# zerenluo123/legged_gym

Hardware: AMD Instinct MI355X
Metric: env-steps/sec (whole node), Go1 rough-terrain 4096 envs/GPU at 1/2/4/8 GPUs (higher is better)
Workload: dtype fp32; 1 GPU; C3 go1_rough: Go1 trimesh curriculum terrain + 187-point height scan, actuator-net history+MLP, PPO 24 steps x 4096 envs/GPU, 5 epochs x 4 minibatches; envs_per_gpu=4096, global_envs=4096, parallelism=dp1

## Files before the change

legged_gym_amd/csrc/lgx_api.hip:

```cpp
#include <math.h>
#include <stddef.h>
#include <stdio.h>
#include <string.h>

#include <new>
#include <string>
#include <vector>

#include "lgx_internal.h"

static thread_local std::string g_err;

static int fail(int code, const char* msg) {
  g_err = msg;
  return code;
}
static int hip_check(hipError_t e, const char* what) {
  if (e == hipSuccess) return 0;
  char buf[256];
  snprintf(buf, sizeof buf, "%s: %s", what, hipGetErrorString(e));
  g_err = buf;
  return LGX_EHIP;
}
int lgx_fail(int code, const char* msg) { return fail(code, msg); }
int lgx_hip_status(const char* what) { return hip_check(hipGetLastError(), what); }
static int launch_check(int rc, const char* what) {
  if (rc == 0) return 0;
  if (rc == -1) return fail(LGX_EINVAL, what);
  return hip_check(hipGetLastError(), what);
}

struct lgx_sim {
  int device;
  bool dense;
  int pp;
  int act_mode;
  int32_t num_points;
  lgx_env_params params;
  lgx_buffers bufs;
  lgx_dev_model* d_model;
  lgx_env_params* d_params;
  const float* draws;
  float* extras_snapshot;
  lgx_priv_args priv;
  lgx_hist_args hist;
  lgx_act_rand_args arand;
  lgx_cmdcur_args ccur;
  hipStream_t aux;
  hipEvent_t aux_in, aux_done;
  bool aux_pending;
  int32_t n_term_rows;
  int32_t profiling;
  int64_t prof_calls;
  std::vector<hipEvent_t> ev[3];
  std::vector<hipEvent_t> pool;
};

static hipEvent_t take_event(lgx_sim* s) {
  if (!s->pool.empty()) { hipEvent_t e = s->pool.back(); s->pool.pop_back(); return e; }
  hipEvent_t e = nullptr;
  if (hipEventCreateWithFlags(&e, hipEventDisableSystemFence) != hipSuccess) return nullptr;
  return e;
}
thread_local lgx_timing_slot lgx_timing;

static int scratch_zeroed(void** slot, size_t bytes, const char* who, const char* what) {
  const std::string w(who), of = std::string("(") + what + ")";
  const bool fresh = !*slot;
  int rc = fresh ? hip_check(hipMalloc(slot, bytes), (w + ": hipMalloc" + of).c_str()) : 0;
// ... 104 lines not shown
  for (int i = 0; i < (dense ? 0 : model->num_points); ++i) {
    int d = model->point_dyn[i];
    int rep = model->point_report[i];
    if (d < 0 || d >= LGX_NUM_DYN) return fail(LGX_EINVAL, "lgx_sim_create: bad point_dyn");
    int lane;
    if (d == 0) {
      if (rep != 0) return fail(LGX_EINVAL, "lgx_sim_create: base points must report on body 0");
      lane = rr++ & 3;
    } else {
      lane = (d - 1) / 3;
      if (rep < 1 + 4 * lane || rep > 4 + 4 * lane) return fail(LGX_EINVAL, "lgx_sim_create: leg point reports on a foreign body");
    }
    if (dm.lane_npts[lane] >= LGX_MAX_LANE_PTS) return fail(LGX_EINVAL, "lgx_sim_create: too many contact points per leg");
    dm.lane_pts[lane][dm.lane_npts[lane]++] = i;
  }
  for (int l = 0; l < 4; ++l) dm.max_lane_npts = dm.lane_npts[l] > dm.max_lane_npts ? dm.lane_npts[l] : dm.max_lane_npts;
  dm.joint_rot_eye = 1;
  for (int j = 0; j < LGX_NUM_DOF; ++j)
    for (int i = 0; i < 9; ++i)
      if (model->joint_rot[j][i] != (i % 4 == 0 ? 1.f : 0.f)) dm.joint_rot_eye = 0;

  int rc = hip_check(hipSetDevice(device), "hipSetDevice");
  if (rc) return rc;
  lgx_sim* s = new (std::nothrow) lgx_sim();
  if (!s) return fail(LGX_ENOMEM, "lgx_sim_create: out of host memory");
  s->device = device;
  s->dense = dense;
  s->pp = lgx_physics_pp(params->num_envs);
  const char* am = getenv("LGX_ACT_OVERLAP");
  s->act_mode = am && *am ? atoi(am) : 2;
  if (s->act_mode < 0 || s->act_mode > 2 || (am && *am && (am[0] < '0' || am[0] > '2' || am[1]))) {
    delete s;
    return fail(LGX_EINVAL, "lgx_sim_create: LGX_ACT_OVERLAP must be 0, 1 or 2");
  }
  s->num_points = model->num_points;
  s->params = *params;
  s->bufs = *bufs;
  s->draws = nullptr;
  s->extras_snapshot = nullptr;
  s->priv = lgx_priv_args{};
  s->hist = lgx_hist_args{};
  s->arand = lgx_act_rand_args{};
  s->ccur = lgx_cmdcur_args{};
  s->aux = nullptr;
  s->aux_in = s->aux_done = nullptr;
  s->aux_pending = false;
  s->profiling = 0;
  s->prof_calls = 0;
  s->n_term_rows = params->num_terms + (params->termination_slot >= 0 ? 1 : 0);
  if ((rc = hip_check(hipMalloc(&s->d_model, sizeof(lgx_dev_model)), "hipMalloc(model)"))) { delete s; return rc; }
  if ((rc = hip_check(hipMalloc(&s->d_params, sizeof(lgx_env_params)), "hipMalloc(params)"))) {
    (void)hipFree(s->d_model); delete s; return rc;
  }
  rc = hip_check(hipMemcpy(s->d_model, &dm, sizeof dm, hipMemcpyHostToDevice), "hipMemcpy(model)");
  if (!rc) rc = hip_check(hipMemcpy(s->d_params, params, sizeof *params, hipMemcpyHostToDevice), "hipMemcpy(params)");
  if (!rc) {
    const int64_t blocks = (params->num_envs + LGX_ENV_BLOCK - 1) / LGX_ENV_BLOCK;
    rc = hip_check(hipMemset(bufs->scratch + blocks * LGX_PARTIAL_STRIDE, 0, sizeof(unsigned int)), "hipMemset(ticket)");
  }
  if (rc) { (void)hipFree(s->d_model); (void)hipFree(s->d_params); delete s; return rc; }
  *out = s;
  return 0;
}

int lgx_sim_destroy(lgx_sim* s) {
  if (!s) return 0;
// ... 238 lines not shown
    pa.n = s->params.num_envs;
    pa.tag = 0u;
    pa.obs = s->bufs.obs;
    pa.hist = s->hist.row;
    pa.hist_width = s->hist.width;
    pa.priv = s->priv.buf;
    pa.priv_width = s->priv.width;
  }
  const int32_t nblocks = (pa.n + LGX_ENV_BLOCK - 1) / LGX_ENV_BLOCK;
  return launch_check(lgx_launch_cmd_curriculum(s->d_params, s->bufs.scratch, nblocks, s->n_term_rows, s->ccur, pa, st),
                      "command curriculum: launch");
}

int lgx_rebind_extras(lgx_sim* s, float* snapshot) {
  if (!s) return fail(LGX_EINVAL, "lgx_rebind_extras: null sim");
  s->extras_snapshot = snapshot;
  return 0;
}

static int join_aux(lgx_sim* s, hipStream_t st) {
  if (!s->aux_pending) return 0;
  return hip_check(hipStreamWaitEvent(st, s->aux_done, 0), "hipStreamWaitEvent(aux)");
}


int lgx_sync_aux(lgx_sim* s, void* stream) {
  if (!s) return fail(LGX_EINVAL, "lgx_sync_aux: null sim");
  return join_aux(s, (hipStream_t)stream);
}

static int physics(lgx_sim* s, int32_t nsub, int32_t from_actions, const float* actions, hipStream_t st, int32_t frozen) {
  if (s->arand.prev)
    return lgx_launch_physics_rand(s->d_model, s->d_params, s->bufs, s->params.num_envs, nsub, from_actions, actions,
                                   st, frozen, s->pp, s->arand);
  return s->dense ? lgx_launch_physics_dense(s->d_model, s->d_params, s->bufs, s->params.num_envs, nsub, from_actions,
                                             actions, st, frozen, s->num_points)
                  : lgx_launch_physics(s->d_model, s->d_params, s->bufs, s->params.num_envs, nsub, from_actions, actions,
                                       st, frozen, s->pp);
}

int lgx_simulate(lgx_sim* s, int32_t n, void* stream) {
  if (!s || n < 0) return fail(LGX_EINVAL, "lgx_simulate: bad arguments");
  if (n == 0) return 0;
  if (int rc = join_aux(s, (hipStream_t)stream)) return rc;
  return launch_check(physics(s, n, 0, nullptr, (hipStream_t)stream, 0), "lgx_simulate: physics launch");
}

int lgx_drive_inputs(lgx_sim* s, const float* actions, void* stream) {
  if (!s) return fail(LGX_EINVAL, "lgx_drive_inputs: null sim");
  if (int rc = join_aux(s, (hipStream_t)stream)) return rc;
  return launch_check(physics(s, s->params.decimation, 1, actions, (hipStream_t)stream, 1), "lgx_drive_inputs: launch");
}

int lgx_ground_contact(lgx_sim* s, const float* points, int32_t n, float* out, void* stream) {
  if (!s || n < 0 || (n > 0 && (!points || !out))) return fail(LGX_EINVAL, "lgx_ground_contact: bad arguments");
  return launch_check(lgx_launch_ground_contact(s->d_params, s->bufs, points, n, out, (hipStream_t)stream),
                      "lgx_ground_contact: launch");
}

int lgx_post_physics(lgx_sim* s, int64_t step, void* stream) {
  if (!s) return fail(LGX_EINVAL, "lgx_post_physics: null sim");
  if (int rc = launch_check(lgx_launch_post_physics(s->d_params, s->bufs, s->params.num_envs, step, s->draws,
                                                    s->extras_snapshot, nullptr, s->priv, s->hist, (hipStream_t)stream),
                            "lgx_post_physics: launch"))
    return rc;
  return command_curriculum(s, step, (hipStream_t)stream, nullptr, 0);
}

static int post_physics_fused(lgx_sim* s, int64_t step, hipStream_t st, bool sample);

int lgx_step(lgx_sim* s, int64_t step, void* stream) { return lgx_step_from(s, nullptr, step, stream); }
// ... 203 lines not shown
```

legged_gym_amd/csrc/lgx_internal.h:

```cpp
#pragma once
#include <hip/hip_ext.h>
#include <hip/hip_runtime.h>

#include "../../include/lgx.h"

#define LGX_MAX_LANE_PTS 24

struct lgx_dev_model {
  lgx_model m;
  int32_t lane_npts[4];
  int32_t max_lane_npts;
  int32_t joint_rot_eye;
  int32_t lane_pts[4][LGX_MAX_LANE_PTS];
  int32_t pad_tail[(4 - (sizeof(lgx_model) / 4 + 6 + 4 * LGX_MAX_LANE_PTS) % 4) % 4];
};

int lgx_launch_ground_contact(const lgx_env_params* dp, const lgx_buffers& b, const float* q, int32_t n, float* o,
                              hipStream_t stream);
int lgx_physics_pp(int32_t n_envs);
int lgx_launch_physics(const lgx_dev_model* dm, const lgx_env_params* dp, const lgx_buffers& b, int32_t n_envs,
                       int32_t nsub, int32_t from_actions, const float* act_src, hipStream_t stream, int32_t frozen,
                       int pp);
struct lgx_act_rand_args {
  const float* kp_scale;
  const float* kd_scale;
  const int32_t* lag;
  float* prev;
};
int lgx_launch_physics_rand(const lgx_dev_model* dm, const lgx_env_params* dp, const lgx_buffers& b, int32_t n_envs,
                            int32_t nsub, int32_t from_actions, const float* act_src, hipStream_t stream,
                            int32_t frozen, int pp, const lgx_act_rand_args& ar);
int lgx_launch_physics_dense(const lgx_dev_model* dm, const lgx_env_params* dp, const lgx_buffers& b, int32_t n_envs,
                             int32_t nsub, int32_t from_actions, const float* act_src, hipStream_t stream,
                             int32_t frozen, int32_t num_points);
struct lgx_priv_args {
  float* buf;
  int32_t width, num_terms;
  uint32_t ids;
  uint32_t pad;
  uint64_t offs_lo, offs_hi;
  float cf_scale, tq_scale;
  __host__ __device__ int id(int t) const { return (int)((ids >> (4 * t)) & 15u); }
  __host__ __device__ int off(int t) const { return (int)(((t < 4 ? offs_lo : offs_hi) >> (16 * (t & 3))) & 0xffffu); }
  void set(int t, int id_, int off_) {
    ids |= (uint32_t)id_ << (4 * t);
    (t < 4 ? offs_lo : offs_hi) |= (uint64_t)off_ << (16 * (t & 3));
  }
};
static_assert(LGX_PRIV_MAX_TERMS <= 8 && LGX_PRIV_COUNT <= 16 && LGX_MAX_PRIV_OBS < 65536, "lgx_priv_args packing");
struct lgx_hist_args {
  float* row;
  const float* prev;
  int32_t* age;
  int32_t frames, frame_width, width;
};
struct lgx_act_launch {
  const float* in;
  float* out;
  int64_t rows;
  const float* w;
  const float* scale;
};
int lgx_launch_post_physics(const lgx_env_params* dp, const lgx_buffers& b, int32_t n_envs, int64_t step,
                            const float* draws, float* extras_snapshot, const lgx_act_launch* act,
// ... 90 lines not shown
```

legged_gym_amd/csrc/lgx_physics.hip:

```cpp
#include <stdlib.h>

#include "lgx_device.h"
#include "lgx_internal.h"

namespace {

struct sv { f3 a, l; };
LGX_DEV sv sv0() { return sv{mk3(0, 0, 0), mk3(0, 0, 0)}; }
LGX_DEV sv add(sv x, sv y) { return sv{x.a + y.a, x.l + y.l}; }
LGX_DEV sv scale(float s, sv x) { return sv{s * x.a, s * x.l}; }
LGX_DEV float dot(sv x, sv y) { return dot(x.a, y.a) + dot(x.l, y.l); }
LGX_DEV sv crm(sv V, sv s) { return sv{cross(V.a, s.a), cross(V.a, s.l) + cross(V.l, s.a)}; }
LGX_DEV sv crf(sv V, sv f) { return sv{cross(V.a, f.a) + cross(V.l, f.l), cross(V.a, f.l)}; }

struct SI { float m; f3 h; float I[6]; };
LGX_DEV SI si_add(const SI& x, const SI& y) {
  SI r; r.m = x.m + y.m; r.h = x.h + y.h;
#pragma unroll
  for (int i = 0; i < 6; ++i) r.I[i] = x.I[i] + y.I[i];
  return r;
}
LGX_DEV sv si_mul(const SI& s, sv v) {
  f3 Ia = mk3(s.I[0] * v.a.x + s.I[3] * v.a.y + s.I[4] * v.a.z, s.I[3] * v.a.x + s.I[1] * v.a.y + s.I[5] * v.a.z,
              s.I[4] * v.a.x + s.I[5] * v.a.y + s.I[2] * v.a.z);
// ... 355 lines not shown
    const int w0 = w[0], w1 = w[LGX_HF_PATCH], w2 = w[1], w3 = w[LGX_HF_PATCH + 1];
    h[0] = w0 >> 8; h[1] = w1 >> 8; h[2] = w2 >> 8; h[3] = w3 >> 8;
    code[0] = w0 & 15; code[1] = w1 & 15; code[2] = w2 & 15; code[3] = w3 & 15;
  } else {
#pragma unroll
    for (int k = 0; k < 4; ++k) {
      const int64_t o = (int64_t)(ci + (k & 1)) * cols + cj + (k >> 1);
      h[k] = B.height_samples[o];
      code[k] = B.hf_trimesh[o];
    }
#pragma unroll
    for (int k = 0; k < 4; ++k) code[k] &= 15;
  }
  f3 v[4];
#pragma unroll
  for (int k = 0; k < 4; ++k) {
    const int da = ca + (k & 1), db = cb + (k >> 1);
    const int dx = ((code[k] * 11) >> 5) - 1, dy = code[k] - 3 * (dx + 1) - 1;
    v[k] = mk3((float)(da - 1 + dx) * hs, (float)(db - 1 + dy) * hs, (float)h[k] * vs);
  }
  const float zmax = fmaxf(fmaxf(v[0].z, v[1].z), fmaxf(v[2].z, v[3].z));
  const float xmin = fminf(fminf(v[0].x, v[1].x), fminf(v[2].x, v[3].x)), xmax = fmaxf(fmaxf(v[0].x, v[1].x), fmaxf(v[2].x, v[3].x));
  const float ymin = fminf(fminf(v[0].y, v[1].y), fminf(v[2].y, v[3].y)), ymax = fmaxf(fmaxf(v[0].y, v[1].y), fmaxf(v[2].y, v[3].y));
  if (p.z - r > zmax || p.x < xmin - r || p.x > xmax + r || p.y < ymin - r || p.y > ymax + r) return;
  tm_tri(q, p, v[0], v[3], v[2]);
  tm_tri(q, p, v[0], v[1], v[3]);
}

LGX_DEV void tm_init(TmQuery& q, f3 p) {
  q.d2 = 3.0e38f; q.cp = p; q.cn = mk3(0.f, 0.f, 1.f);
  q.top = -3.0e38f; q.tn = mk3(0.f, 0.f, 1.f);
}

LGX_DEV float tm_finish(const TmQuery& q, f3 p, float r, f3* n) {
  const bool inside = p.z < q.top;
  const float d = sqrtf(q.d2);
  if (d > 1e-7f) {
    const float inv = ph_rcp(d);
    *n = inside ? inv * (q.cp - p) : inv * (p - q.cp);
  } else {
    f3 c = q.top > -1e30f ? q.tn : q.cn;
    c = (c.z < 0.f ? -1.f : 1.f) / fmaxf(sqrtf(dot(c, c)), 1e-30f) * c;
    *n = c;
  }
  return inside ? r + d : r - d;
}

LGX_DEV bool tm_near(const lgx_env_params* __restrict__ P, const lgx_buffers& B, f3 p, float r, int i, int j,
                     const int32_t* hpatch, int pi0, int pj0) {
  int hv[16], cd[16];
  tm_block(B, i, j, hpatch, pi0, pj0, hv, cd);
  int hmax = hv[0];
#pragma unroll
  for (int k = 1; k < 16; ++k) hmax = max(hmax, hv[k]);
  return !(p.z - r > (float)hmax * P->vertical_scale);
}

LGX_DEV unsigned tm_keep(const lgx_env_params* __restrict__ P, const lgx_buffers& B, f3 p, float r, int i, int j,
                         const int32_t* hpatch, int pi0, int pj0, f3* pl) {
  const float hs = P->horizontal_scale, vs = P->vertical_scale;
  const int rows = B.hf_rows, cols = B.hf_cols;
  int hv[16], cd[16];
  tm_block(B, i, j, hpatch, pi0, pj0, hv, cd);
  int hmax = hv[0];
#pragma unroll
  for (int k = 1; k < 16; ++k) hmax = max(hmax, hv[k]);
// ... 84 lines not shown
              h11 = (float)(q11 >> 8) * vs;
  const float fu = clampf(u - (float)i, 0.f, 1.f), fv = clampf(v - (float)j, 0.f, 1.f);
  float gx, gy, h;
  if (fu >= fv) { gx = (h10 - h00) * ihs; gy = (h11 - h10) * ihs; h = h00 + fu * (h10 - h00) + fv * (h11 - h10); }
  else          { gx = (h11 - h01) * ihs; gy = (h01 - h00) * ihs; h = h00 + fv * (h01 - h00) + fu * (h11 - h01); }
  const float inv = ph_rsqrt(gx * gx + gy * gy + 1.0f);
  *n = mk3(-gx * inv, -gy * inv, inv);
  return (h - p.z) * n->z + r;
}

LGX_DEV float ground_contact(const lgx_env_params* __restrict__ P, const lgx_buffers& B, f3 p, float r, f3* n,
                             const int32_t* patch, int pi0, int pj0) {
  bool defer;
  const float d = ground_cell(P, B, p, r, n, patch, pi0, pj0, &defer);
  if (!defer) return d;
  int i, j;
  tm_cell(P, B, p, &i, &j);
  return trimesh_depth(P, B, p, r, i, j, n, patch, pi0, pj0);
}

LGX_DEV void wave_lds_sync() {
  __builtin_amdgcn_fence(__ATOMIC_RELEASE, "wavefront");
  __builtin_amdgcn_wave_barrier();
  __builtin_amdgcn_fence(__ATOMIC_ACQUIRE, "wavefront");
}

}

#define MAX_LANE_PTS LGX_MAX_LANE_PTS
#ifndef LGX_PHYS_WAVES_PER_SIMD
#define LGX_PHYS_WAVES_PER_SIMD 1
#endif
#define HIST_STRIDE 31

template <int PP>
LGX_DEV float psum(float v) {
  if (PP == 4) return row_quads_sum(v);
  if (PP >= 2) v += lane_xor4(v);
  if (PP >= 4) v += lane_xor8(v);
  if (PP >= 8) v += __shfl_xor(v, 16);
  return v;
}

#define PHYS_KP(k, j) (RAND ? arow[k] : M->kp[j])
#define PHYS_KD(k, j) (RAND ? arow[3 + (k)] : M->kd[j])
#define PHYS_PG(k, j) (RAND ? arow[k] : P->p_gains[j])
#define PHYS_DG(k, j) (RAND ? arow[3 + (k)] : P->d_gains[j])
#define PHYS_AE(k) (RAND ? ae_lag[k] : act[k])
LGX_DEV lgx_act_rand_args act_rand_of() { return lgx_act_rand_args{nullptr, nullptr, nullptr, nullptr}; }
LGX_DEV lgx_act_rand_args act_rand_of(const lgx_act_rand_args& a) { return a; }

template <int PP, typename... AR>
__global__ void __launch_bounds__(64 * PP, LGX_PHYS_WAVES_PER_SIMD)
lgx_physics_kernel(const lgx_dev_model* __restrict__ DMg, const lgx_env_params* __restrict__ P, lgx_buffers B,
                   int32_t nsub, int32_t from_actions, const float* __restrict__ act_src, int32_t frozen, AR... ar) {
  static_assert(sizeof...(AR) <= 1, "at most the actuator tables");
  constexpr bool RAND = sizeof...(AR) == 1;
  constexpr int PHYS_BLOCK = 64 * PP;
  constexpr int LPE = 4 * PP;
  constexpr int SLOTS = (MAX_LANE_PTS + PP - 1) / PP;
  constexpr int ENVS = 16;
  __shared__ lgx_dev_model smodel;
  __shared__ float4 slot_state[SLOTS][PHYS_BLOCK];
  __shared__ float4 geo_p[SLOTS][PHYS_BLOCK];
  __shared__ float4 geo_n[SLOTS][PHYS_BLOCK];
  __shared__ float hist_lds[ENVS * 4 * HIST_STRIDE];
  __shared__ float leg_kin[ENVS * 4][3][12];
  __shared__ float leg_sys[ENVS * 4][36];
  __shared__ float env_com[ENVS][40];
  __shared__ int32_t hf_patch[ENVS][LGX_HF_PATCH * LGX_HF_PATCH];
  __shared__ int32_t hf_org[ENVS][2];
  __shared__ uint32_t tm_q[PP][64 * SLOTS];
  {
    static_assert(sizeof(lgx_dev_model) % 16 == 0, "the model is staged in 16-byte units");
    const int4* src = reinterpret_cast<const int4*>(DMg);
    int4* dst = reinterpret_cast<int4*>(&smodel);
    for (int i = threadIdx.x; i < (int)(sizeof(lgx_dev_model) / 16); i += PHYS_BLOCK) dst[i] = src[i];
    __syncthreads();
  }
  const lgx_dev_model* DM = &smodel;
  const lgx_model* M = &smodel.m;
  const int tid = threadIdx.x;
  const int gl = blockIdx.x * PHYS_BLOCK + tid;
  const int e = gl / LPE;
  const int lie = gl % LPE;
  const int eb = tid / LPE;
  const int leg = lie & 3;
  const int pl = lie >> 2;
  const bool lane0 = leg == 0;
  const bool owner = pl == 0;
  const int N = P->num_envs;
  const bool valid = e < N;
  const int ec = valid ? e : N - 1;

  LGX_CLK_DECL(12)
#ifdef LGX_PHASE_CLOCK
  unsigned lgx_bodies[4] = {0u, 0u, 0u, 0u};
#endif
  const float dt = M->sim_dt;
  const float* rs = B.root_states + (int64_t)ec * 13;
  f3 pos = mk3(rs[0], rs[1], rs[2]);
  float qx = rs[3], qy = rs[4], qz = rs[5], qw = rs[6];
  f3 vlin = mk3(rs[7], rs[8], rs[9]);
  f3 wang = mk3(rs[10], rs[11], rs[12]);
  float th[3], thd[3], tgt[3], act[3];
// ... 323 lines not shown
      for (int sl = 0; sl < SLOTS; ++sl) {
        if (sl >= nslots) break;
        const bool act = pl + PP * sl < npts;
        const int pi = slot_pt[sl];
        const int db = slot_db[sl];
        const int k = db == 0 ? -1 : (db - 1) % 3;
        const float* fr = db == 0 ? ecom + 27 : kin + 12 * k;
        m33 R;
#pragma unroll
        for (int i = 0; i < 9; ++i) R.a[i] = fr[i];
        f3 ol = db == 0 ? mk3(0, 0, 0) : mk3(fr[9], fr[10], fr[11]);
        f3 Pp = ol + mul(R, mk3(M->point_pos[pi][0], M->point_pos[pi][1], M->point_pos[pi][2]));
        const float rad = M->point_radius[pi];
        f3 n;
        bool defer;
        const float depth = ground_cell(P, B, Pp + pos, rad, &n, patch, pi0, pj0, &defer);
        defer = defer && act;
        const uint64_t m = __ballot(defer);
        if (defer) {
          tm_q[wv][qn + __popcll(m & below)] = (uint32_t)(sl << 6 | ln);
          geo_p[sl][tid] = make_float4(Pp.x, Pp.y, Pp.z, rad);
          geo_n[sl][tid] = make_float4(0.f, 0.f, 1.f, (float)pi);
        } else if (act) {
          slot_state[sl][tid] = make_float4(depth > 0.f ? 1.f : 0.f, 0.f, 0.f, 0.f);
          if (depth > 0.f) {
            const f3 Pc = Pp - rad * n;
            geo_p[sl][tid] = make_float4(Pc.x, Pc.y, Pc.z, depth);
            geo_n[sl][tid] = make_float4(n.x, n.y, n.z, (float)pi);
          }
        }
        qn += __popcll(m);
      }
      LGX_CLK(8);
      if (qn > 0) {
        wave_lds_sync();
        const bool cull1 = qn > 16;
        int qn2 = 0;
        for (int q0 = 0; q0 < qn; q0 += 64) {
          const int q = q0 + ln;
          uint32_t ent = 0;
          unsigned keep = 0;
          if (q < qn) {
            ent = tm_q[wv][q];
            const int sl2 = (ent >> 6) & 1023, t = (wv << 6) | (ent & 63), e2 = t / LPE;
            const float4 g = geo_p[sl2][t];
            const f3 pw = mk3(g.x, g.y, g.z) + mk3(env_com[e2][36], env_com[e2][37], env_com[e2][38]);
            const int32_t* hp = use_patch ? hf_patch[e2] : nullptr;
            const int o0 = use_patch ? hf_org[e2][0] : 0, o1 = use_patch ? hf_org[e2][1] : 0;
            int i, j;
            tm_cell(P, B, pw, &i, &j);
            if (cull1) {
              f3 pl3;
              keep = tm_keep(P, B, pw, g.w, i, j, hp, o0, o1, &pl3);
            } else {
              keep = tm_near(P, B, pw, g.w, i, j, hp, o0, o1) ? 0x1ffu : 0u;
            }
            if (!keep) slot_state[sl2][t] = make_float4(0.f, 0.f, 0.f, 0.f);
          }
          const uint64_t m = __ballot(keep != 0);
          if (keep) tm_q[wv][qn2 + __popcll(m & below)] = ent | keep << 16;
          qn2 += __popcll(m);
        }
        wave_lds_sync();
        LGX_CLK(9);
#ifdef LGX_PHASE_CLOCK
        lgx_clk_acc[11] += (uint64_t)qn * 1000 + qn2;
#endif
        if (qn2 <= 8) {
          const int grp = ln >> 4, g = ln & 15;
          for (int q0 = 0; q0 < qn2; q0 += 4) {
            const int q = min(q0 + grp, qn2 - 1);
            const uint32_t ent = tm_q[wv][q];
            const int sl2 = (ent >> 6) & 1023, t = (wv << 6) | (ent & 63), e2 = t / LPE;
            const float4 gp = geo_p[sl2][t];
            const f3 Pp = mk3(gp.x, gp.y, gp.z);
            const f3 pw = Pp + mk3(env_com[e2][36], env_com[e2][37], env_com[e2][38]);
            const int32_t* hp = use_patch ? hf_patch[e2] : nullptr;
            const int o0 = use_patch ? hf_org[e2][0] : 0, o1 = use_patch ? hf_org[e2][1] : 0;
            int i, j;
            tm_cell(P, B, pw, &i, &j);
            const f3 pl3 = tm_local(P, pw, i, j);
            TmQuery tq;
            tm_init(tq, pl3);
            if (g < 9 && ((ent >> (16 + g)) & 1u))
              tm_cell_tris(tq, P, B, pl3, gp.w, i, j, (g * 11) >> 5, g - 3 * ((g * 11) >> 5), hp, o0, o1);
            int cd2 = g, ctop = g;
            tm_combine_step<1>(tq, cd2, ctop);
            tm_combine_step<2>(tq, cd2, ctop);
            tm_combine_step<4>(tq, cd2, ctop);
            tm_combine_step<8>(tq, cd2, ctop);
            if (g == 0 && q0 + grp < qn2) {
              f3 n;
              const float depth = tm_finish(tq, pl3, gp.w, &n);
              slot_state[sl2][t] = make_float4(depth > 0.f ? 1.f : 0.f, 0.f, 0.f, 0.f);
              if (depth > 0.f) {
                const f3 Pc = Pp - gp.w * n;
                geo_p[sl2][t] = make_float4(Pc.x, Pc.y, Pc.z, depth);
                geo_n[sl2][t] = make_float4(n.x, n.y, n.z, geo_n[sl2][t].w);
              }
            }
          }
        } else {
          for (int q0 = 0; q0 < qn2; q0 += 64) {
            const int q = q0 + ln;
            if (q < qn2) {
              const uint32_t ent = tm_q[wv][q];
              const int sl2 = (ent >> 6) & 1023, t = (wv << 6) | (ent & 63), e2 = t / LPE;
              const float4 gp = geo_p[sl2][t];
              const f3 Pp = mk3(gp.x, gp.y, gp.z);
              const f3 pw = Pp + mk3(env_com[e2][36], env_com[e2][37], env_com[e2][38]);
              int i, j;
              tm_cell(P, B, pw, &i, &j);
              f3 n;
              const float depth = tm_visit(P, B, tm_local(P, pw, i, j), gp.w, i, j, ent >> 16, &n,
                                           use_patch ? hf_patch[e2] : nullptr, use_patch ? hf_org[e2][0] : 0,
                                           use_patch ? hf_org[e2][1] : 0);
              slot_state[sl2][t] = make_float4(depth > 0.f ? 1.f : 0.f, 0.f, 0.f, 0.f);
              if (depth > 0.f) {
                const f3 Pc = Pp - gp.w * n;
                geo_p[sl2][t] = make_float4(Pc.x, Pc.y, Pc.z, depth);
                geo_n[sl2][t] = make_float4(n.x, n.y, n.z, geo_n[sl2][t].w);
              }
            }
          }
        }
      }
      wave_lds_sync();
    }
    uint32_t own_act = 0;
    {
      float sx[SLOTS];
#pragma unroll
      for (int sl = 0; sl < SLOTS; ++sl) sx[sl] = slot_state[sl][tid].x;
#pragma unroll
      for (int sl = 0; sl < SLOTS; ++sl)
        own_act |= ((unsigned)(pl + PP * sl < npts) & (unsigned)(sx[sl] != 0.f)) << sl;
    }
    LGX_CLK(10);
    float xb[6];
    f3 xl;
    for (int pass = 0; pass < 2; ++pass) {
      LegSys L;
#pragma unroll
      for (int i = 0; i < 21; ++i) L.Ap[i] = 0.f;
#pragma unroll
      for (int i = 0; i < 6; ++i) { L.rb[i] = 0.f; L.B[i][0] = L.B[i][1] = L.B[i][2] = 0.f; }
#pragma unroll
      for (int i = 0; i < 6; ++i) L.D[i] = 0.f;
      L.rl[0] = L.rl[1] = L.rl[2] = 0.f;
      uint32_t w = own_act;
#pragma unroll 1
      for (int trip = 0; trip < SLOTS; ++trip) {
        if (__ballot(w != 0u) == 0) break;
        const bool on = w != 0u;
        const int sl = on ? __builtin_ctz(w) : 0;
        w &= w - 1;
        const float4 st = slot_state[sl][tid];
        const float4 gp = geo_p[sl][tid], gn = geo_n[sl][tid];
        const bool use = on && st.x != 0.f;
        const int db = M->point_dyn[use ? (int)gn.w : 0];
// ... 154 lines not shown
#pragma unroll
  for (int r = 0; r < 4; ++r) {
    float* d = cfo + (1 + 4 * leg + r) * 3;
    d[0] = cf_leg[r].x; d[1] = cf_leg[r].y; d[2] = cf_leg[r].z;
  }
  if (use_hist) {
    float* h = B.act_hist + (int64_t)e * 120 + leg * 30;
#pragma unroll
    for (int i = 0; i < 30; i += 2) *reinterpret_cast<float2*>(h + i) = make_float2(hist[i], hist[i + 1]);
  }
  if (lane0) {
    cfo[0] = cf_base.x; cfo[1] = cf_base.y; cfo[2] = cf_base.z;
    float* ro = B.root_states + (int64_t)e * 13;
    ro[0] = pos.x; ro[1] = pos.y; ro[2] = pos.z;
    ro[3] = qx; ro[4] = qy; ro[5] = qz; ro[6] = qw;
    ro[7] = vlin.x; ro[8] = vlin.y; ro[9] = vlin.z;
    ro[10] = wang.x; ro[11] = wang.y; ro[12] = wang.z;
  }
  LGX_CLK(7);
  LGX_CLK_PRINT("physics", 12)
#if defined(LGX_PHASE_CLOCK) && !defined(LGX_PHASE_CLOCK_BUF)
  if (LGX_CLK_WHO)
    printf("physics bodies: b=%d pass0=%u pass1=%u classify=%u report=%u\n", (int)blockIdx.x, lgx_bodies[0],
           lgx_bodies[1], lgx_bodies[2], lgx_bodies[3]);
#elif defined(LGX_PHASE_CLOCK)
  (void)lgx_bodies;
#endif
}

#ifdef LGX_PHYSICS_RAND

int lgx_launch_physics_rand(const lgx_dev_model* dm, const lgx_env_params* dp, const lgx_buffers& b, int32_t n_envs,
                            int32_t nsub, int32_t from_actions, const float* act_src, hipStream_t stream,
                            int32_t frozen, int ppx, const lgx_act_rand_args& ar) {
  if (!ar.prev) return -1;
  if (!act_src) act_src = b.actions;
  const int blocks = (n_envs + 15) / 16;
  if (ppx == 8)
    LGX_LAUNCH((lgx_physics_kernel<8, lgx_act_rand_args>), dim3(blocks), dim3(512), 0, stream, dm, dp, b, nsub,
               from_actions, act_src, frozen, ar);
  else if (ppx == 4)
    LGX_LAUNCH((lgx_physics_kernel<4, lgx_act_rand_args>), dim3(blocks), dim3(256), 0, stream, dm, dp, b, nsub,
               from_actions, act_src, frozen, ar);
  else if (ppx == 2)
    LGX_LAUNCH((lgx_physics_kernel<2, lgx_act_rand_args>), dim3(blocks), dim3(128), 0, stream, dm, dp, b, nsub,
               from_actions, act_src, frozen, ar);
  else
    LGX_LAUNCH((lgx_physics_kernel<1, lgx_act_rand_args>), dim3(blocks), dim3(64), 0, stream, dm, dp, b, nsub,
               from_actions, act_src, frozen, ar);
  return hipGetLastError() == hipSuccess ? 0 : -2;
}

#else

__global__ void lgx_ground_contact_kernel(const lgx_env_params* __restrict__ P, lgx_buffers B, const float4* __restrict__ q,
                                          int32_t n, float4* __restrict__ o) {
  const int k = blockIdx.x * blockDim.x + threadIdx.x;
  if (k >= n) return;
  const float4 v = q[k];
  f3 nn;
  const float d = ground_contact(P, B, mk3(v.x, v.y, v.z), v.w, &nn, nullptr, 0, 0);
  o[k] = make_float4(d, nn.x, nn.y, nn.z);
}

int lgx_launch_ground_contact(const lgx_env_params* dp, const lgx_buffers& b, const float* q, int32_t n, float* o,
                              hipStream_t stream) {
  if (n <= 0) return 0;
  hipLaunchKernelGGL(lgx_ground_contact_kernel, dim3((n + 255) / 256), dim3(256), 0, stream, dp, b,
                     reinterpret_cast<const float4*>(q), n, reinterpret_cast<float4*>(o));
  return hipGetLastError() == hipSuccess ? 0 : -2;
}

int lgx_physics_pp(int32_t n_envs) {
  (void)n_envs;
  const char* force = getenv("LGX_PHYS_PP");
  const int f = force ? atoi(force) : 0;
  return (f == 1 || f == 2 || f == 4 || f == 8) ? f : 4;
}

int lgx_launch_physics(const lgx_dev_model* dm, const lgx_env_params* dp, const lgx_buffers& b, int32_t n_envs,
                       int32_t nsub, int32_t from_actions, const float* act_src, hipStream_t stream, int32_t frozen,
                       int ppx) {
  if (!act_src) act_src = b.actions;
  const int blocks = (n_envs + 15) / 16;
  if (ppx == 8)
    LGX_LAUNCH(lgx_physics_kernel<8>, dim3(blocks), dim3(512), 0, stream, dm, dp, b, nsub, from_actions, act_src, frozen);
  else if (ppx == 4)
    LGX_LAUNCH(lgx_physics_kernel<4>, dim3(blocks), dim3(256), 0, stream, dm, dp, b, nsub, from_actions, act_src, frozen);
  else if (ppx == 2)
    LGX_LAUNCH(lgx_physics_kernel<2>, dim3(blocks), dim3(128), 0, stream, dm, dp, b, nsub, from_actions, act_src, frozen);
  else
    LGX_LAUNCH(lgx_physics_kernel<1>, dim3(blocks), dim3(64), 0, stream, dm, dp, b, nsub, from_actions, act_src, frozen);
  return hipGetLastError() == hipSuccess ? 0 : -2;
}


namespace {

constexpr int DN = 18;
constexpr int DCF = 3 * DN + 3 + 3 + 1 + 1 + 3 + 3;

struct DenseLds {
  float R[LGX_NUM_DYN][9], o[LGX_NUM_DYN][3], S[LGX_NUM_DOF][6], I6[LGX_NUM_DYN][36];
  float H[DN * DN], M[DN * DN];
  float V[LGX_NUM_DYN][6], A[LGX_NUM_DYN][6], F[LGX_NUM_DYN][6];
  float ICroot[4][36], Froot[4][6];
  float Cb[DN], g[DN], Hu[DN], r[DN], u[DN], u2[DN];
  float th[12], thd[12], tgt[12], tex[12], Dimp[12];
  float root[13];
  int impl[12];
  int nc;
};

struct DenseContacts {
  float (*J)[3 * DN];
  float (*P)[3];
  float (*n)[3];
  float* depth;
  float* mu;
  float (*fs)[3];
  float (*f)[3];
  int* body;
  int* report;
  int* stat;
};
// ... 479 lines not shown
      const f3 q = mk3(L.root[3], L.root[4], L.root[5]);
      const float qw = L.root[6];
      const f3 wq = cross(w, q);
      float dq[4] = {0.5f * (qw * w.x + wq.x), 0.5f * (qw * w.y + wq.y), 0.5f * (qw * w.z + wq.z), -0.5f * dot(w, q)};
      float qq[4] = {q.x + dt * dq[0], q.y + dt * dq[1], q.z + dt * dq[2], qw + dt * dq[3]};
      const float qn = 1.0f / sqrtf(qq[0] * qq[0] + qq[1] * qq[1] + qq[2] * qq[2] + qq[3] * qq[3]);
      L.root[3] = qq[0] * qn; L.root[4] = qq[1] * qn; L.root[5] = qq[2] * qn; L.root[6] = qq[3] * qn;
      L.root[7] = v.x; L.root[8] = v.y; L.root[9] = v.z;
      L.root[10] = w.x; L.root[11] = w.y; L.root[12] = w.z;
    }
    __syncthreads();
  }
  if (lane < 12) {
    B.dof_state[(int64_t)e * 24 + 2 * lane] = L.th[lane];
    B.dof_state[(int64_t)e * 24 + 2 * lane + 1] = L.thd[lane];
    if (ctrl != LGX_CTRL_POS_DRIVE && nsub > 0) B.torques[(int64_t)e * 12 + lane] = L.tex[lane];
  }
  if (lane < 13) B.root_states[(int64_t)e * 13 + lane] = L.root[lane];
}

static int lgx_physics_dense_lds(int32_t num_points) { return num_points * (DCF + 3) * 4; }

int lgx_launch_physics_dense(const lgx_dev_model* dm, const lgx_env_params* dp, const lgx_buffers& b, int32_t n_envs,
                             int32_t nsub, int32_t from_actions, const float* act_src, hipStream_t stream,
                             int32_t frozen, int32_t num_points) {
  if (!act_src) act_src = b.actions;
  const int cap = num_points > 0 ? num_points : 1;
  LGX_LAUNCH(lgx_physics_dense_kernel, dim3(n_envs), dim3(64), lgx_physics_dense_lds(cap), stream, dm, dp, b, nsub,
             from_actions, act_src, frozen, cap);
  return hipGetLastError() == hipSuccess ? 0 : -2;
}

#ifdef LGX_PHASE_CLOCK_BUF
extern "C" int lgx_debug_clock(unsigned long long* out, int32_t nblocks) {
  return hipMemcpyFromSymbol(out, HIP_SYMBOL(lgx_clk_buf), (size_t)min(nblocks, LGX_CLK_MAXB) * 14 * 8, 0,
                             hipMemcpyDeviceToHost) == hipSuccess ? 0 : -1;
}
#endif

#endif
```

Before: 6.230 million env-steps/s.

## Add packed per-triangle stage-2 trimesh contact path with tunable dispatch thresholds

Adds a packed stage-2 mode for trimesh contact queries. The surviving candidate triangles of all queries are compacted into one wave-wide list, each lane tests one triangle, the partial results go to LDS, and each owning query then merges its range. The first-stage cull threshold drops from 16 to 4 queries, the rows-form threshold drops from 8 to 4, and packed is chosen automatically for up to 16 surviving queries. A new env var forces a given form, and optional timing buffers are added. The aim is better lane use when few queries survive, at the cost of more LDS, extra wave syncs and register pressure.

```diff
diff --git a/legged_gym_amd/csrc/lgx_api.hip b/legged_gym_amd/csrc/lgx_api.hip
--- a/legged_gym_amd/csrc/lgx_api.hip
+++ b/legged_gym_amd/csrc/lgx_api.hip
@@ -35,6 +35,7 @@
   bool dense;
   int pp;
   int act_mode;
+  int tm_mode;
   int32_t num_points;
   lgx_env_params params;
   lgx_buffers bufs;
@@ -205,6 +206,13 @@
   if (s->act_mode < 0 || s->act_mode > 2 || (am && *am && (am[0] < '0' || am[0] > '2' || am[1]))) {
     delete s;
     return fail(LGX_EINVAL, "lgx_sim_create: LGX_ACT_OVERLAP must be 0, 1 or 2");
+  }
+  const char* tm = getenv("LGX_TM_STAGE2");
+  s->tm_mode = !tm || !*tm ? LGX_TM_AUTO : !strcmp(tm, "rows") ? LGX_TM_ROWS : !strcmp(tm, "lane") ? LGX_TM_LANE
+               : !strcmp(tm, "packed") ? LGX_TM_PACKED : -1;
+  if (s->tm_mode < 0) {
+    delete s;
+    return fail(LGX_EINVAL, "lgx_sim_create: LGX_TM_STAGE2 must be rows, lane or packed");
   }
   s->num_points = model->num_points;
   s->params = *params;
@@ -509,11 +517,11 @@
 static int physics(lgx_sim* s, int32_t nsub, int32_t from_actions, const float* actions, hipStream_t st, int32_t frozen) {
   if (s->arand.prev)
     return lgx_launch_physics_rand(s->d_model, s->d_params, s->bufs, s->params.num_envs, nsub, from_actions, actions,
-                                   st, frozen, s->pp, s->arand);
+                                   st, frozen, s->pp, s->tm_mode, s->arand);
   return s->dense ? lgx_launch_physics_dense(s->d_model, s->d_params, s->bufs, s->params.num_envs, nsub, from_actions,
                                              actions, st, frozen, s->num_points)
                   : lgx_launch_physics(s->d_model, s->d_params, s->bufs, s->params.num_envs, nsub, from_actions, actions,
-                                       st, frozen, s->pp);
+                                       st, frozen, s->pp, s->tm_mode);
 }
 
 int lgx_simulate(lgx_sim* s, int32_t n, void* stream) {
diff --git a/legged_gym_amd/csrc/lgx_internal.h b/legged_gym_amd/csrc/lgx_internal.h
--- a/legged_gym_amd/csrc/lgx_internal.h
+++ b/legged_gym_amd/csrc/lgx_internal.h
@@ -18,9 +18,10 @@
 int lgx_launch_ground_contact(const lgx_env_params* dp, const lgx_buffers& b, const float* q, int32_t n, float* o,
                               hipStream_t stream);
 int lgx_physics_pp(int32_t n_envs);
+enum { LGX_TM_AUTO = 0, LGX_TM_ROWS = 1, LGX_TM_LANE = 2, LGX_TM_PACKED = 3 };
 int lgx_launch_physics(const lgx_dev_model* dm, const lgx_env_params* dp, const lgx_buffers& b, int32_t n_envs,
                        int32_t nsub, int32_t from_actions, const float* act_src, hipStream_t stream, int32_t frozen,
-                       int pp);
+                       int pp, int32_t tm_mode);
 struct lgx_act_rand_args {
   const float* kp_scale;
   const float* kd_scale;
@@ -29,7 +30,7 @@
 };
 int lgx_launch_physics_rand(const lgx_dev_model* dm, const lgx_env_params* dp, const lgx_buffers& b, int32_t n_envs,
                             int32_t nsub, int32_t from_actions, const float* act_src, hipStream_t stream,
-                            int32_t frozen, int pp, const lgx_act_rand_args& ar);
+                            int32_t frozen, int pp, int32_t tm_mode, const lgx_act_rand_args& ar);
 int lgx_launch_physics_dense(const lgx_dev_model* dm, const lgx_env_params* dp, const lgx_buffers& b, int32_t n_envs,
                              int32_t nsub, int32_t from_actions, const float* act_src, hipStream_t stream,
                              int32_t frozen, int32_t num_points);
diff --git a/legged_gym_amd/csrc/lgx_physics.hip b/legged_gym_amd/csrc/lgx_physics.hip
--- a/legged_gym_amd/csrc/lgx_physics.hip
+++ b/legged_gym_amd/csrc/lgx_physics.hip
@@ -411,6 +411,41 @@
   q.top = -3.0e38f; q.tn = mk3(0.f, 0.f, 1.f);
 }
 
+LGX_DEV void tm_cell_verts(const lgx_env_params* __restrict__ P, const lgx_buffers& B, int i, int j, int ca, int cb,
+                           const int32_t* hpatch, int pi0, int pj0, f3* v) {
+#pragma clang fp contract(off)
+  const float hs = P->horizontal_scale, vs = P->vertical_scale;
+  const int cols = B.hf_cols;
+  const int ci = i - 1 + ca, cj = j - 1 + cb;
+  int h[4], code[4];
+  if (hpatch && (unsigned)(ci - pi0) < LGX_HF_PATCH - 1 && (unsigned)(cj - pj0) < LGX_HF_PATCH - 1) {
+    const int32_t* w = hpatch + (ci - pi0) * LGX_HF_PATCH + (cj - pj0);
+    const int w0 = w[0], w1 = w[LGX_HF_PATCH], w2 = w[1], w3 = w[LGX_HF_PATCH + 1];
+    h[0] = w0 >> 8; h[1] = w1 >> 8; h[2] = w2 >> 8; h[3] = w3 >> 8;
+    code[0] = w0 & 15; code[1] = w1 & 15; code[2] = w2 & 15; code[3] = w3 & 15;
+  } else {
+#pragma unroll
+    for (int k = 0; k < 4; ++k) {
+      const int64_t o = (int64_t)(ci + (k & 1)) * cols + cj + (k >> 1);
+      h[k] = B.height_samples[o];
+      code[k] = B.hf_trimesh[o];
+    }
+#pragma unroll
+    for (int k = 0; k < 4; ++k) code[k] &= 15;
+  }
+#pragma unroll
+  for (int k = 0; k < 4; ++k) {
+    const int da = ca + (k & 1), db = cb + (k >> 1);
+    const int dx = ((code[k] * 11) >> 5) - 1, dy = code[k] - 3 * (dx + 1) - 1;
+    v[k] = mk3((float)(da - 1 + dx) * hs, (float)(db - 1 + dy) * hs, (float)h[k] * vs);
+  }
+}
+
+LGX_DEV void tm_merge(TmQuery& q, const TmQuery& o) {
+  if (o.d2 < q.d2) { q.d2 = o.d2; q.cp = o.cp; q.cn = o.cn; }
+  if (o.top > q.top) { q.top = o.top; q.tn = o.tn; }
+}
+
 LGX_DEV float tm_finish(const TmQuery& q, f3 p, float r, f3* n) {
   const bool inside = p.z < q.top;
   const float d = sqrtf(q.d2);
@@ -561,6 +596,18 @@
 #define LGX_PHYS_WAVES_PER_SIMD 1
 #endif
 #define HIST_STRIDE 31
+#ifndef LGX_TM_CULL1_QN
+#define LGX_TM_CULL1_QN 4
+#endif
+#ifndef LGX_TM_ROWS_QN2
+#define LGX_TM_ROWS_QN2 4
+#endif
+#ifndef LGX_TM_PACKED_QN2
+#define LGX_TM_PACKED_QN2 16
+#endif
+#ifdef LGX_PHASE_CLOCK_BUF
+static __device__ unsigned lgx_tmq_buf[LGX_CLK_MAXB][8][4][4];
+#endif
 
 template <int PP>
 LGX_DEV float psum(float v) {
@@ -582,7 +629,8 @@
 template <int PP, typename... AR>
 __global__ void __launch_bounds__(64 * PP, LGX_PHYS_WAVES_PER_SIMD)
 lgx_physics_kernel(const lgx_dev_model* __restrict__ DMg, const lgx_env_params* __restrict__ P, lgx_buffers B,
-                   int32_t nsub, int32_t from_actions, const float* __restrict__ act_src, int32_t frozen, AR... ar) {
+                   int32_t nsub, int32_t from_actions, const float* __restrict__ act_src, int32_t frozen,
+                   int32_t tm_mode, AR... ar) {
   static_assert(sizeof...(AR) <= 1, "at most the actuator tables");
   constexpr bool RAND = sizeof...(AR) == 1;
   constexpr int PHYS_BLOCK = 64 * PP;
@@ -600,6 +648,8 @@
   __shared__ int32_t hf_patch[ENVS][LGX_HF_PATCH * LGX_HF_PATCH];
   __shared__ int32_t hf_org[ENVS][2];
   __shared__ uint32_t tm_q[PP][64 * SLOTS];
+  __shared__ uint32_t tm_tl[PP][64];
+  __shared__ float tm_rec[PP][11][64];
   {
     static_assert(sizeof(lgx_dev_model) % 16 == 0, "the model is staged in 16-byte units");
     const int4* src = reinterpret_cast<const int4*>(DMg);
@@ -989,9 +1039,14 @@
         qn += __popcll(m);
       }
       LGX_CLK(8);
+#ifdef LGX_PHASE_CLOCK_BUF
+      const uint64_t lgx_tmq_t0 = clock64();
+      uint64_t lgx_tmq_t1 = lgx_tmq_t0;
+      int lgx_tmq_form = 0, lgx_tmq_qn2 = 0;
+#endif
       if (qn > 0) {
         wave_lds_sync();
-        const bool cull1 = qn > 16;
+        const bool cull1 = tm_mode == LGX_TM_PACKED || qn > LGX_TM_CULL1_QN;
         int qn2 = 0;
         for (int q0 = 0; q0 < qn; q0 += 64) {
           const int q = q0 + ln;
@@ -1023,7 +1078,114 @@
 #ifdef LGX_PHASE_CLOCK
         lgx_clk_acc[11] += (uint64_t)qn * 1000 + qn2;
 #endif
-        if (qn2 <= 8) {
+#ifdef LGX_PHASE_CLOCK_BUF
+        lgx_tmq_t1 = clock64();
+        lgx_tmq_qn2 = qn2;
+#endif
+        const bool rows = tm_mode == LGX_TM_ROWS || (tm_mode == LGX_TM_AUTO && qn2 <= LGX_TM_ROWS_QN2);
+        const bool packed = tm_mode == LGX_TM_PACKED ||
+                            (tm_mode == LGX_TM_AUTO && cull1 && !rows && qn2 <= LGX_TM_PACKED_QN2);
+#ifdef LGX_PHASE_CLOCK_BUF
+        lgx_tmq_form = packed ? 3 : rows ? 1 : 2;
+#endif
+        if (packed) {
+          for (int b0 = 0; b0 < qn2; b0 += 64) {
+            const uint32_t ent = tm_q[wv][min(b0 + ln, qn2 - 1)];
+            const unsigned keep = b0 + ln < qn2 ? (ent >> 16) & 0x1ffu : 0u;
+            const int nc = __popc(keep);
+            int start = 0, total = 0;
+#pragma unroll
+            for (int b = 0; b < 4; ++b) {
+              const uint64_t m = __ballot((nc >> b) & 1);
+              start += __popcll(m & below) << (b + 1);
+              total += __popcll(m) << (b + 1);
+            }
+            const int end = start + 2 * nc;
+            for (int r0 = 0; r0 < total;) {
+              const uint64_t cut = __ballot(start < r0 + 64 && end > r0 + 64);
+              const int rend = cut ? __builtin_amdgcn_readlane(start, (int)__builtin_ctzll(cut)) : min(total, r0 + 64);
+              const bool mine = start >= r0 && end <= rend && keep != 0u;
+              {
+                unsigned rem = mine ? keep : 0u;
+                int nxt = start - r0;
+                for (;;) {
+                  const bool on = rem != 0u;
+                  if (__ballot(on) == 0) break;
+                  if (on) {
+                    const uint32_t w = (uint32_t)(ln << 5 | __builtin_ctz(rem) << 1);
+                    tm_tl[wv][nxt] = w;
+                    tm_tl[wv][nxt + 1] = w | 1u;
+                    rem &= rem - 1;
+                    nxt += 2;
+                  }
+                }
+              }
+              wave_lds_sync();
+              {
+                const uint32_t tr = tm_tl[wv][min(ln, rend - r0 - 1)];
+                const uint32_t ent3 = tm_q[wv][b0 + (int)(tr >> 5)];
+                const int sl3 = (ent3 >> 6) & 1023, t3 = (wv << 6) | (ent3 & 63), e3 = t3 / LPE;
+                const float4 g3 = geo_p[sl3][t3];
+                const f3 pw3 = mk3(g3.x, g3.y, g3.z) + mk3(env_com[e3][36], env_com[e3][37], env_com[e3][38]);
+                const int32_t* hp = use_patch ? hf_patch[e3] : nullptr;
+                const int o0 = use_patch ? hf_org[e3][0] : 0, o1 = use_patch ? hf_org[e3][1] : 0;
+                int i3, j3;
+                tm_cell(P, B, pw3, &i3, &j3);
+                const f3 p3 = tm_local(P, pw3, i3, j3);
+                const int c = (tr >> 1) & 15, ca = (c * 11) >> 5;
+                f3 v[4];
+                tm_cell_verts(P, B, i3, j3, ca, c - 3 * ca, hp, o0, o1, v);
+                const bool second = (tr & 1u) != 0u;
+                TmQuery tq;
+                tm_init(tq, p3);
+                tm_tri(tq, p3, v[0], second ? v[1] : v[3], second ? v[3] : v[2]);
+                const float w[11] = {tq.d2, tq.cp.x, tq.cp.y, tq.cp.z, tq.cn.x, tq.cn.y, tq.cn.z, tq.top, tq.tn.x, tq.tn.y, tq.tn.z};
+#pragma unroll
+                for (int k = 0; k < 11; ++k) tm_rec[wv][k][ln] = w[k];
+              }
+              wave_lds_sync();
+              const int sl2 = (ent >> 6) & 1023, t = (wv << 6) | (ent & 63), e2 = t / LPE;
+              const float4 gp = geo_p[sl2][t];
+              const f3 Pp = mk3(gp.x, gp.y, gp.z);
+              const f3 pw = Pp + mk3(env_com[e2][36], env_com[e2][37], env_com[e2][38]);
+              int i, j;
+              tm_cell(P, B, pw, &i, &j);
+              const f3 pl3 = tm_local(P, pw, i, j);
+              TmQuery run;
+              tm_init(run, pl3);
+              int p = mine ? start - r0 : 0;
+              const int pe = mine ? end - r0 : 0;
+              for (;;) {
+                const bool on = p < pe;
+                if (__ballot(on) == 0) break;
+                const int pc = on ? p : 0;
+                float w[11];
+#pragma unroll
+                for (int k = 0; k < 11; ++k) w[k] = tm_rec[wv][k][pc];
+                if (on) {
+                  TmQuery o;
+                  o.d2 = w[0]; o.cp = mk3(w[1], w[2], w[3]);
+                  o.cn = mk3(w[4], w[5], w[6]); o.top = w[7];
+                  o.tn = mk3(w[8], w[9], w[10]);
+                  tm_merge(run, o);
+                }
+                ++p;
+              }
+              if (mine) {
+                f3 n;
+                const float depth = tm_finish(run, pl3, gp.w, &n);
+                slot_state[sl2][t] = make_float4(depth > 0.f ? 1.f : 0.f, 0.f, 0.f, 0.f);
+                if (depth > 0.f) {
+                  const f3 Pc = Pp - gp.w * n;
+                  geo_p[sl2][t] = make_float4(Pc.x, Pc.y, Pc.z, depth);
+                  geo_n[sl2][t] = make_float4(n.x, n.y, n.z, geo_n[sl2][t].w);
+                }
+              }
+              wave_lds_sync();
+              r0 = rend;
+            }
+          }
+        } else if (rows) {
           const int grp = ln >> 4, g = ln & 15;
           for (int q0 = 0; q0 < qn2; q0 += 4) {
             const int q = min(q0 + grp, qn2 - 1);
@@ -1083,6 +1245,15 @@
         }
       }
       wave_lds_sync();
+#ifdef LGX_PHASE_CLOCK_BUF
+      if (ln == 0 && blockIdx.x < LGX_CLK_MAXB) {
+        unsigned* r = lgx_tmq_buf[blockIdx.x][wv & 7][s & 3];
+        r[0] = (unsigned)qn << 16 | (unsigned)lgx_tmq_qn2;
+        r[1] = (unsigned)(lgx_tmq_t1 - lgx_tmq_t0);
+        r[2] = (unsigned)(clock64() - lgx_tmq_t1);
+        r[3] = (unsigned)lgx_tmq_form;
+      }
+#endif
     }
     uint32_t own_act = 0;
     {
@@ -1303,22 +1474,22 @@
 
 int lgx_launch_physics_rand(const lgx_dev_model* dm, const lgx_env_params* dp, const lgx_buffers& b, int32_t n_envs,
                             int32_t nsub, int32_t from_actions, const float* act_src, hipStream_t stream,
-                            int32_t frozen, int ppx, const lgx_act_rand_args& ar) {
+                            int32_t frozen, int ppx, int32_t tm_mode, const lgx_act_rand_args& ar) {
   if (!ar.prev) return -1;
   if (!act_src) act_src = b.actions;
   const int blocks = (n_envs + 15) / 16;
   if (ppx == 8)
     LGX_LAUNCH((lgx_physics_kernel<8, lgx_act_rand_args>), dim3(blocks), dim3(512), 0, stream, dm, dp, b, nsub,
-               from_actions, act_src, frozen, ar);
+               from_actions, act_src, frozen, tm_mode, ar);
   else if (ppx == 4)
     LGX_LAUNCH((lgx_physics_kernel<4, lgx_act_rand_args>), dim3(blocks), dim3(256), 0, stream, dm, dp, b, nsub,
-               from_actions, act_src, frozen, ar);
+               from_actions, act_src, frozen, tm_mode, ar);
   else if (ppx == 2)
     LGX_LAUNCH((lgx_physics_kernel<2, lgx_act_rand_args>), dim3(blocks), dim3(128), 0, stream, dm, dp, b, nsub,
-               from_actions, act_src, frozen, ar);
+               from_actions, act_src, frozen, tm_mode, ar);
   else
     LGX_LAUNCH((lgx_physics_kernel<1, lgx_act_rand_args>), dim3(blocks), dim3(64), 0, stream, dm, dp, b, nsub,
-               from_actions, act_src, frozen, ar);
+               from_actions, act_src, frozen, tm_mode, ar);
   return hipGetLastError() == hipSuccess ? 0 : -2;
 }
 
@@ -1351,17 +1522,17 @@
 
 int lgx_launch_physics(const lgx_dev_model* dm, const lgx_env_params* dp, const lgx_buffers& b, int32_t n_envs,
                        int32_t nsub, int32_t from_actions, const float* act_src, hipStream_t stream, int32_t frozen,
-                       int ppx) {
+                       int ppx, int32_t tm_mode) {
   if (!act_src) act_src = b.actions;
   const int blocks = (n_envs + 15) / 16;
   if (ppx == 8)
-    LGX_LAUNCH(lgx_physics_kernel<8>, dim3(blocks), dim3(512), 0, stream, dm, dp, b, nsub, from_actions, act_src, frozen);
+    LGX_LAUNCH(lgx_physics_kernel<8>, dim3(blocks), dim3(512), 0, stream, dm, dp, b, nsub, from_actions, act_src, frozen, tm_mode);
   else if (ppx == 4)
-    LGX_LAUNCH(lgx_physics_kernel<4>, dim3(blocks), dim3(256), 0, stream, dm, dp, b, nsub, from_actions, act_src, frozen);
+    LGX_LAUNCH(lgx_physics_kernel<4>, dim3(blocks), dim3(256), 0, stream, dm, dp, b, nsub, from_actions, act_src, frozen, tm_mode);
   else if (ppx == 2)
-    LGX_LAUNCH(lgx_physics_kernel<2>, dim3(blocks), dim3(128), 0, stream, dm, dp, b, nsub, from_actions, act_src, frozen);
+    LGX_LAUNCH(lgx_physics_kernel<2>, dim3(blocks), dim3(128), 0, stream, dm, dp, b, nsub, from_actions, act_src, frozen, tm_mode);
   else
-    LGX_LAUNCH(lgx_physics_kernel<1>, dim3(blocks), dim3(64), 0, stream, dm, dp, b, nsub, from_actions, act_src, frozen);
+    LGX_LAUNCH(lgx_physics_kernel<1>, dim3(blocks), dim3(64), 0, stream, dm, dp, b, nsub, from_actions, act_src, frozen, tm_mode);
   return hipGetLastError() == hipSuccess ? 0 : -2;
 }
 
@@ -1907,6 +2078,10 @@
 }
 
 #ifdef LGX_PHASE_CLOCK_BUF
+extern "C" int lgx_debug_tmq(unsigned* out, int32_t nblocks) {
+  return hipMemcpyFromSymbol(out, HIP_SYMBOL(lgx_tmq_buf), (size_t)min(nblocks, LGX_CLK_MAXB) * 8 * 4 * 4 * 4, 0,
+                             hipMemcpyDeviceToHost) == hipSuccess ? 0 : -1;
+}
 extern "C" int lgx_debug_clock(unsigned long long* out, int32_t nblocks) {
   return hipMemcpyFromSymbol(out, HIP_SYMBOL(lgx_clk_buf), (size_t)min(nblocks, LGX_CLK_MAXB) * 14 * 8, 0,
                              hipMemcpyDeviceToHost) == hipSuccess ? 0 : -1;
```

Measured after the change: 6.312 million env-steps/s, median of 6. +1.3%, better.
